# blachlylab/fade

Measured on NVIDIA B200. Metric: annotate_reads_per_sec, higher is better.
Workload: dtype int16

## Files before the change

### fade_b200/csrc/emu/emu.cu

```cuda
#include <cstdio>
#include <cstdlib>
#include <cstring>
#include <vector>
#include "../sw_core.cuh"

using namespace fade;

namespace {

template <int R>
struct ThreadState {
    uint32_t H[R], E[R], qs[R];
    uint32_t hu_prev, fout, M;
};

template <int R>
int align_pair(const uint8_t *qa, int qlen_a, const uint8_t *ta, int tlen_a,
               const uint8_t *qb, int qlen_b, const uint8_t *tb, int tlen_b,
               const SwConsts &k, int extra_blocks, int tagged, int32_t min_length,
               uint32_t clipl_a, uint32_t clipr_a, uint32_t clipl_b, uint32_t clipr_b,
               AlnOut *out_a, AlnOut *out_b)
{
    const int rows = FG * R;
    if (qlen_a > rows || qlen_b > rows) return -1;
    const int tmax = tlen_a > tlen_b ? tlen_a : tlen_b;
    const int nblk = num_blocks(tmax) + extra_blocks;
    const int TW = FBLK * nblk + FG + 1;
    std::vector<uint16_t> tw(TW);
    for (int idx = 0; idx < TW; ++idx) {
        const int j = idx - FG;
        const int ca = (j >= 0 && j < tlen_a) ? ta[j] : C_TPAD;
        const int cb = (j >= 0 && j < tlen_b) ? tb[j] : C_TPAD;
        tw[idx] = (uint16_t)t_sel(ca, cb);
    }
    std::vector<uint8_t> qc(rows);
    std::vector<ThreadState<R>> st(FG);
    for (int g = 0; g < FG; ++g)
        for (int r = 0; r < R; ++r) {
            const int i = g * R + r;
            const int ca = i < qlen_a ? qa[i] : C_QPAD;
            const int cb = i < qlen_b ? qb[i] : C_QPAD;
            st[g].qs[r] = q_sel(ca, cb);
            qc[i] = (uint8_t)(ca | (cb << 4));
        }
    auto init_state = [&](ThreadState<R> &s) {
        for (int r = 0; r < R; ++r) { s.H[r] = 0; s.E[r] = k.neg_o; }
        s.hu_prev = 0; s.fout = k.neg_o; s.M = 0;
    };
    for (int g = 0; g < FG; ++g) init_state(st[g]);

    const int CW = ck_words<R>();
    std::vector<uint32_t> ck((size_t)nblk * FG * CW);
    LaneCtl ctl[2];
    memset(ctl, 0, sizeof(ctl));
    uint32_t Mprev[FG];
    for (int g = 0; g < FG; ++g) Mprev[g] = 0;
    for (int c = 0; c < nblk; ++c) {
        for (int u = 0; u < FBLK; ++u) {
            const int t = c * FBLK + u;
            uint32_t hu[FG], fin[FG];
            for (int g = 0; g < FG; ++g) {
                hu[g] = g == 0 ? 0u : st[g - 1].H[R - 1];
                fin[g] = g == 0 ? k.neg_o : st[g - 1].fout;
            }
            for (int g = 0; g < FG; ++g) {
                const uint32_t ts = tw[t - g + FG];
                const uint32_t hd = st[g].hu_prev;
                fill_step<R>(st[g].H, st[g].E, st[g].qs, st[g].M, ts, hd, fin[g], st[g].fout, k);
                st[g].hu_prev = hu[g];
            }
        }
        for (int g = 0; g < FG; ++g) {
            uint32_t *p = &ck[((size_t)c * FG + g) * CW];
            for (int r = 0; r < R; ++r) { p[r] = st[g].H[r]; p[R + r] = st[g].E[r]; }
            p[2 * R] = st[g].hu_prev;
            p[2 * R + 1] = st[g].fout;
            if (st[g].M != Mprev[g]) {
                if (lane_lo(st[g].M) != lane_lo(Mprev[g])) ctl[0].blk[g] = c;
                if (lane_hi(st[g].M) != lane_hi(Mprev[g])) ctl[1].blk[g] = c;
                Mprev[g] = st[g].M;
            }
        }
    }
    for (int g = 0; g < FG; ++g) { ctl[0].best[g] = lane_lo(st[g].M); ctl[1].best[g] = lane_hi(st[g].M); }

    ctl_init(ctl[0], qlen_a, tlen_a);
    ctl_init(ctl[1], qlen_b, tlen_b);
    constexpr int RW = trace_words<R>();
    std::vector<uint32_t> tr((size_t)tile_words<R>());
    const bool tg = (tagged & 1) && k.tagged_ok;
    int guard = 0;
    bool first_iter = true;
    while (ctl[0].phase != 2 || ctl[1].phase != 2) {
        if (++guard > 4 * nblk + 16) return -2;
        int blk[2];
        for (int L = 0; L < 2; ++L) blk[L] = (ctl[L].phase != 2 && ctl[L].next_blk >= 0) ? ctl[L].next_blk : 0;
        bool scan[2][FG];
        for (int L = 0; L < 2; ++L)
            for (int g = 0; g < FG; ++g) scan[L][g] = (ctl_scanmask(ctl[L]) >> g) & 1u;
        for (int g = 0; g < FG; ++g) {
            ThreadState<R> s0, s1;
            init_state(s0); init_state(s1);
            auto load = [&](ThreadState<R> &s, int b) {
                if (b == 0) return;
                const uint32_t *p = &ck[((size_t)(b - 1) * FG + g) * CW];
                for (int r = 0; r < R; ++r) { s.H[r] = p[r]; s.E[r] = p[R + r]; }
                s.hu_prev = p[2 * R]; s.fout = p[2 * R + 1];
            };
            load(s0, blk[0]); load(s1, blk[1]);
            auto mix = [&](uint32_t a, uint32_t b) {
                const uint32_t w = (a & 0xffffu) | (b & 0xffff0000u);
                return tg ? to_tagged(w) : w;
            };
            for (int r = 0; r < R; ++r) { st[g].H[r] = mix(s0.H[r], s1.H[r]); st[g].E[r] = mix(s0.E[r], s1.E[r]); }
            st[g].hu_prev = mix(s0.hu_prev, s1.hu_prev);
            st[g].fout = mix(s0.fout, s1.fout);
        }
        const uint32_t f_top = tg ? k.neg_o16 : k.neg_o;
        const int mul = tg ? 16 : 1;
        bool found[2][FG];
        for (int L = 0; L < 2; ++L) for (int g = 0; g < FG; ++g) found[L][g] = false;
        for (int u = 0; u < FBLK; ++u) {
            const int t0 = blk[0] * FBLK + u, t1 = blk[1] * FBLK + u;
            uint32_t hu[FG], fin[FG];
            for (int g = 0; g < FG; ++g) {
                hu[g] = g == 0 ? 0u : st[g - 1].H[R - 1];
                fin[g] = g == 0 ? f_top : st[g - 1].fout;
            }
            for (int g = 0; g < FG; ++g) {
                const uint32_t ts = (tw[t0 - g + FG] & 0x00ffu) | (tw[t1 - g + FG] & 0xff00u);
                uint32_t cmax = 0;
                uint32_t trw[RW];
                if (tg) trace_step_tagged<R>(st[g].H, st[g].E, st[g].qs, ts, st[g].hu_prev, fin[g], st[g].fout, k, trw, cmax);
                else trace_step_plain<R>(st[g].H, st[g].E, st[g].qs, ts, st[g].hu_prev, fin[g], st[g].fout, k, trw, cmax);
                st[g].hu_prev = hu[g];
                for (int w = 0; w < RW; ++w) tr[(size_t)tile_index<R>(u, g, w)] = trw[w];
                for (int L = 0; L < 2; ++L) {
                    if (!scan[L][g] || found[L][g]) continue;
                    const int cm = L == 0 ? lane_lo(cmax) : lane_hi(cmax);
                    if (cm != ctl[L].S * mul) continue;
                    for (int r = 0; r < R; ++r) {
                        const int hv = L == 0 ? lane_lo(st[g].H[r]) : lane_hi(st[g].H[r]);
                        if (hv == ctl[L].S * mul) {
                            found[L][g] = true;
                            ctl[L].fj[g] = (L == 0 ? t0 : t1) - g;
                            ctl[L].fr[g] = r;
                            break;
                        }
                    }
                }
            }
        }
        for (int L = 0; L < 2; ++L)
            for (int g = 0; g < FG; ++g)
                if (scan[L][g] && !found[L][g]) return -3;
        const bool so0 = (tagged & 4) && ctl[0].phase == 0 && first_iter, so1 = (tagged & 4) && ctl[1].phase == 0 && first_iter;
        ctl_advance<R>(ctl[0], so0 ? nullptr : tr.data(), 0, StagedAcc{ tw.data(), qc.data(), 0 }, k);
        ctl_advance<R>(ctl[1], so1 ? nullptr : tr.data(), 1, StagedAcc{ tw.data(), qc.data(), 1 }, k);
        first_iter = false;
    }
    finalize_result(ctl[0], *out_a, 0, clipl_a, clipr_a, min_length);
    finalize_result(ctl[1], *out_b, 1, clipl_b, clipr_b, min_length);
    return 0;
}

}

extern "C" int fadeemu_align_pair(int R, const uint8_t *qa, int qlen_a, const uint8_t *ta, int tlen_a,
                                  const uint8_t *qb, int qlen_b, const uint8_t *tb, int tlen_b,
                                  int open, int extend, int match, int mismatch, int extra_blocks,
                                  int tagged, int min_length, const uint32_t *clips ,
                                  AlnOut *out_a, AlnOut *out_b)
{
    SwConsts k = make_consts(open, extend, match, mismatch);
    k.shortcut = (tagged & 2) ? 0 : 1;
#define CASE(RR)                                                                                   \
    case RR:                                                                                       \
        return align_pair<RR>(qa, qlen_a, ta, tlen_a, qb, qlen_b, tb, tlen_b, k, extra_blocks,    \
                              tagged, min_length, clips[0], clips[1], clips[2], clips[3], out_a, out_b);
    switch (R) {
        CASE(1) CASE(2) CASE(3) CASE(5) CASE(13) CASE(19) CASE(25) CASE(32) CASE(38)
    default: return -10;
    }
#undef CASE
}

extern "C" int fadeemu_comp_code_of_nt16(int nib) { return comp_code_of_nt16(nib); }
extern "C" uint32_t fadeemu_prmt(uint32_t a, uint32_t b, uint32_t s) { return prmt_sx(a, b, s); }
extern "C" int fadeemu_sizeof_alnout(void) { return (int)sizeof(AlnOut); }
```

### fade_b200/csrc/kernels.cu

```cuda
#include "kernels.cuh"
#include <algorithm>
#include <cstdio>
#include <cstdlib>

namespace fade {

namespace {

constexpr unsigned FULL = 0xffffffffu;

#define FADE_SMALL_KERNEL __launch_bounds__(128, 16)


__device__ __forceinline__ uint32_t stage_targets(const KernelArgs &a, const AlnDesc &da, const AlnDesc &db, int g,
                                                  int step0, int nsteps, uint16_t *tw)
{
    const int TW = nsteps + FG + 1;
    uint32_t w = 0;
    for (int idx = g; idx < TW; idx += FG) {
        const int j = step0 + idx - FG;
        int ca = C_TPAD, cb = C_TPAD;
        if (j >= 0 && j < da.tlen) ca = ref_code(a.ref.planes, da.gstart + j);
        if (j >= 0 && j < db.tlen) cb = ref_code(a.ref.planes, db.gstart + j);
        w |= (ca == C_WILD ? 1u : 0u) | (cb == C_WILD ? 2u : 0u);
        tw[idx] = (uint16_t)t_sel(ca, cb);
    }
    return w;
}

template <int R>
__device__ __forceinline__ void stage_pair(const KernelArgs &a, const AlnDesc &da, const AlnDesc &db,
                                           int g, int nblk, uint16_t *tw, uint32_t (&qs)[R],
                                           uint8_t *qc, uint32_t &wild)
{
    uint32_t w = stage_targets(a, da, db, g, 0, FBLK * min(nblk, FILL_CHUNK_BLOCKS), tw);
    const uint8_t *sa = a.seq + da.seq_off, *sb = a.seq + db.seq_off;
#pragma unroll
    for (int r = 0; r < R; ++r) {
        const int i = g * R + r;
        int ca = C_QPAD, cb = C_QPAD;
        if (i < da.qlen) ca = rc_query_code(sa, da.qlen, i);
        if (i < db.qlen) cb = rc_query_code(sb, db.qlen, i);
        w |= (ca == C_WILD ? 1u : 0u) | (cb == C_WILD ? 2u : 0u);
        qs[r] = q_sel(ca, cb);
        if (qc) qc[i] = (uint8_t)(ca | (cb << 4));
    }
    wild = w;
}

__device__ __forceinline__ AlnDesc load_desc(const KernelArgs &a, int idx)
{
    AlnDesc d;
    if (idx < a.n_aln) d = a.aln[idx];
    else { d.gstart = 0; d.seq_off = 0; d.tlen = 0; d.qlen = 0; d.clip_left = d.clip_right = 0; d.read = -1; d.pad = 0; }
    return d;
}

template <int R>
__global__ void __launch_bounds__(FILL_THREADS, (R <= 19 ? 5 : 1)) sw_fill_kernel(const KernelArgs a)
{
    extern __shared__ __align__(16) unsigned char smem_raw[];
    const int lane = threadIdx.x & 31, wib = threadIdx.x >> 5;
    const int g = lane & (FG - 1), q = lane >> 3;
    const int w = blockIdx.x * (FILL_THREADS / 32) + wib;
    if (w >= a.n_items) return;
    const WarpItem item = a.items[w];
    const int ia = item.first + 2 * q, ib = ia + 1;
    const AlnDesc da = load_desc(a, ia), db = load_desc(a, ib);
    uint16_t *tw = reinterpret_cast<uint16_t *>(smem_raw) + (size_t)(wib * 4 + q) * a.tw_stride;
    const int nblk = item.nblk;
    const SwConsts k = a.k;

    uint32_t H[R], E[R], qs[R];
    uint32_t wild;
    stage_pair<R>(a, da, db, g, nblk, tw, qs, nullptr, wild);
#pragma unroll
    for (int r = 0; r < R; ++r) { H[r] = 0u; E[r] = k.neg_o; }
    uint32_t hu_prev = 0u, fout = k.neg_o, M = 0u, Mprev = 0u;
    int blk_lo = 0, blk_hi = 0;
    __syncwarp();

    constexpr int CW = ck_words<R>();
    uint32_t *ckw = a.ck + item.ck_off + lane;
    const uint16_t *twp = tw + (FG - g);
    const int nsteps = item.nsteps;
    for (int c = 0; c < nblk; ++c) {
        if (c > 0 && (c % FILL_CHUNK_BLOCKS) == 0) {
            __syncwarp();
            wild |= stage_targets(a, da, db, g, c * FBLK, FBLK * min(nblk - c, FILL_CHUNK_BLOCKS), tw);
            twp = tw + (FG - g) - c * FBLK;
            __syncwarp();
        }
        const int ulim = min(FBLK, nsteps - c * FBLK);
#pragma unroll 2
        for (int u = 0; u < ulim; ++u) {
            const int t = c * FBLK + u;
            uint32_t hu = __shfl_up_sync(FULL, H[R - 1], 1, FG);
            uint32_t fin = __shfl_up_sync(FULL, fout, 1, FG);
            if (g == 0) { hu = 0u; fin = k.neg_o; }
            const uint32_t ts = twp[t];
            fill_step<R>(H, E, qs, M, ts, hu_prev, fin, fout, k);
            hu_prev = hu;
        }
        if (c + 1 < nblk) {
            uint32_t *p = ckw + (size_t)c * CW * 32;
#pragma unroll
            for (int r = 0; r < R; ++r) { p[r * 32] = H[r]; p[(R + r) * 32] = E[r]; }
            p[(2 * R) * 32] = hu_prev;
            p[(2 * R + 1) * 32] = fout;
        }
        if (M != Mprev) {
            if ((M ^ Mprev) & 0xffffu) blk_lo = c;
            if ((M ^ Mprev) >> 16) blk_hi = c;
            Mprev = M;
        }
    }
    a.fillres[(size_t)w * 32 + lane] = make_uint2(M, (uint32_t)blk_lo | ((uint32_t)blk_hi << 16));
    if ((wild & 1u) && ia < a.n_aln) a.aln_flags[ia] = 1u;
    if ((wild & 2u) && ib < a.n_aln) a.aln_flags[ib] = 1u;
}

__device__ __forceinline__ unsigned long long pack_req(int aln, int blk, uint32_t scanmask)
{
    return (unsigned long long)(uint32_t)aln | ((unsigned long long)(uint32_t)(blk & 0xffff) << 32) |
           ((unsigned long long)(scanmask & 0xffu) << 48);
}

struct GlobalAcc {
    const uint8_t *seq;
    int qlen;
    RefPlanes planes;
    int64_t gstart;
    __device__ __forceinline__ int qcode(int i) const { return rc_query_code(seq, qlen, i); }
    __device__ __forceinline__ int tcode(int j) const { return ref_code(planes, gstart + j); }
};

template <int R>
__global__ void FADE_SMALL_KERNEL trace_init_kernel(const KernelArgs a)
{
    for (int aln = blockIdx.x * blockDim.x + threadIdx.x; aln < a.n_aln; aln += gridDim.x * blockDim.x) {
        a.out[aln].read = -1;
        a.out[aln].flags = 0x80000000u;
        if (a.aln_flags[aln] & 1u) continue;
        const AlnDesc d = a.aln[aln];
        LaneCtl &c = a.state[aln];
        const int w = aln >> 3, q = (aln & 7) >> 1, half = aln & 1;
        const uint2 *fr = a.fillres + (size_t)w * 32 + q * FG;
        for (int g = 0; g < FG; ++g) {
            const uint2 v = fr[g];
            c.best[g] = half ? lane_hi(v.x) : lane_lo(v.x);
            c.blk[g] = half ? (int)(v.y >> 16) : (int)(v.y & 0xffffu);
        }
        ctl_init(c, d.qlen, d.tlen);
        if (c.phase != 2 && a.tags_only && !score_may_accept(c.S, d.clip_left, d.clip_right, a.min_length)) {
            AlnOut o;
            o.score = c.S; o.end_query = o.end_ref = o.beg_query = o.beg_ref = 0; o.n_ops = 0;
            o.flags = R_ALIGNED | R_SCORE_ONLY; o.read = d.read;
            for (int k = 0; k < OPS_CAP; ++k) o.ops[k] = 0;
            a.out[aln] = o;
        } else if (c.phase == 2) {
            AlnOut o;
            finalize_result(c, o, d.read, d.clip_left, d.clip_right, a.min_length);
            a.out[aln] = o;
        } else {
            const unsigned slot = atomicAdd(&a.qcount[0], 1u);
            a.queue[0][slot] = pack_req(aln, c.next_blk, ctl_scanmask(c));
        }
    }
}

template <int R, int MODE>
__device__ __forceinline__ void replay_round(const KernelArgs &a, int round, unsigned warp0, unsigned nwarps,
                                             uint16_t (*tws_all)[40])
{
    constexpr bool TAGGED = MODE == 0;
    constexpr bool SCAN_ONLY = MODE == 2;
    constexpr int RW = trace_words<R>();
    constexpr int CW = ck_words<R>();
    constexpr int MUL = TAGGED ? 16 : 1;
    const int lane = threadIdx.x & 31, wib = threadIdx.x >> 5;
    const int g = lane & (FG - 1), q = lane >> 3;
    const int rin = round & 1;
    const unsigned cnt = a.qcount[rin];
    const unsigned long long *queue = a.queue[rin];
    const unsigned npairs = (cnt + 1u) >> 1;
    const unsigned nquads = (npairs + 3u) >> 2;
    const SwConsts k = a.k;
    const uint32_t e_init = TAGGED ? k.neg_o16 : k.neg_o;
    uint16_t *tws = tws_all[wib * 4 + q];
    for (unsigned quad = warp0; quad < nquads; quad += nwarps) {
        const unsigned pair = quad * 4u + (unsigned)q;
        int aln[2], blk[2], half[2], S[2];
        uint32_t smask[2];
        AlnDesc d[2];
        const uint32_t *ckp[2];
#pragma unroll
        for (int L = 0; L < 2; ++L) {
            const unsigned ri = pair * 2u + (unsigned)L;
            if (ri < cnt) {
                const unsigned long long rq = queue[ri];
                aln[L] = (int)(uint32_t)(rq & 0xffffffffu);
                blk[L] = (int)((rq >> 32) & 0xffffu);
                smask[L] = (uint32_t)((rq >> 48) & 0xffu);
                d[L] = a.aln[aln[L]];
                const WarpItem it = a.items[aln[L] >> 3];
                ckp[L] = a.ck + it.ck_off + (((aln[L] & 7) >> 1) * FG + g);
                half[L] = aln[L] & 1;
                S[L] = a.state[aln[L]].S * MUL;
            } else {
                aln[L] = -1; blk[L] = 0; smask[L] = 0; half[L] = 0; S[L] = -1; ckp[L] = a.ck;
                d[L].gstart = 0; d[L].seq_off = 0; d[L].tlen = 0; d[L].qlen = 0;
            }
        }
        uint32_t H[R], E[R], qs[R], hu_prev, fout;
        {
            const uint32_t *p0 = ckp[0] + (size_t)(blk[0] > 0 ? blk[0] - 1 : 0) * CW * 32;
            const uint32_t *p1 = ckp[1] + (size_t)(blk[1] > 0 ? blk[1] - 1 : 0) * CW * 32;
            const bool z0 = blk[0] == 0, z1 = blk[1] == 0;
            const int sh0 = half[0] * 16, sh1 = half[1] * 16;
            auto mix = [&](uint32_t w0, uint32_t w1) {
                const uint32_t w = ((w0 >> sh0) & 0xffffu) | ((w1 >> sh1) << 16);
                return TAGGED ? to_tagged(w) : w;
            };
#pragma unroll
            for (int r = 0; r < R; ++r) {
                H[r] = mix(z0 ? 0u : p0[r * 32], z1 ? 0u : p1[r * 32]);
                E[r] = mix(z0 ? k.neg_o : p0[(R + r) * 32], z1 ? k.neg_o : p1[(R + r) * 32]);
            }
            hu_prev = mix(z0 ? 0u : p0[(2 * R) * 32], z1 ? 0u : p1[(2 * R) * 32]);
            fout = mix(z0 ? k.neg_o : p0[(2 * R + 1) * 32], z1 ? k.neg_o : p1[(2 * R + 1) * 32]);
        }
        {
            const uint8_t *s0 = a.seq + d[0].seq_off, *s1 = a.seq + d[1].seq_off;
#pragma unroll
            for (int r = 0; r < R; ++r) {
                const int i = g * R + r;
                const int ca = i < d[0].qlen ? rc_query_code(s0, d[0].qlen, i) : C_QPAD;
                const int cb = i < d[1].qlen ? rc_query_code(s1, d[1].qlen, i) : C_QPAD;
                qs[r] = q_sel(ca, cb);
            }
            __syncwarp();
            for (int x = g; x < FBLK + FG - 1; x += FG) {
                const int j0 = blk[0] * FBLK - (FG - 1) + x, j1 = blk[1] * FBLK - (FG - 1) + x;
                const int ca = (j0 >= 0 && j0 < d[0].tlen) ? ref_code(a.ref.planes, d[0].gstart + j0) : C_TPAD;
                const int cb = (j1 >= 0 && j1 < d[1].tlen) ? ref_code(a.ref.planes, d[1].gstart + j1) : C_TPAD;
                tws[x] = (uint16_t)t_sel(ca, cb);
            }
            __syncwarp();
        }
        uint32_t *tile = a.tiles + (size_t)pair * tile_words<R>();
        const bool store = aln[0] >= 0;
        bool need0 = (smask[0] >> g) & 1u, need1 = (smask[1] >> g) & 1u;
        const uint16_t *twp = tws + (FG - 1 - g);
        for (int u = 0; u < FBLK; ++u) {
            uint32_t hu = __shfl_up_sync(FULL, H[R - 1], 1, FG);
            uint32_t fin = __shfl_up_sync(FULL, fout, 1, FG);
            if (g == 0) { hu = 0u; fin = e_init; }
            const uint32_t ts = twp[u];
            uint32_t cmax = 0u;
            if (SCAN_ONLY) {
                fill_step<R>(H, E, qs, cmax, ts, hu_prev, fin, fout, k);
            } else {
                uint32_t trw[RW];
                if (TAGGED) trace_step_tagged<R>(H, E, qs, ts, hu_prev, fin, fout, k, trw, cmax);
                else trace_step_plain<R>(H, E, qs, ts, hu_prev, fin, fout, k, trw, cmax);
                if (store) {
#pragma unroll
                    for (int w = 0; w < RW; ++w) tile[tile_index<R>(u, g, w)] = trw[w];
                }
            }
            hu_prev = hu;
            if (need0 && lane_lo(cmax) == S[0]) {
                need0 = false;
                int fr = 0;
#pragma unroll
                for (int r = R - 1; r >= 0; --r) if (lane_lo(H[r]) == S[0]) fr = r;
                a.state[aln[0]].fj[g] = blk[0] * FBLK + u - g;
                a.state[aln[0]].fr[g] = fr;
            }
            if (need1 && lane_hi(cmax) == S[1]) {
                need1 = false;
                int fr = 0;
#pragma unroll
                for (int r = R - 1; r >= 0; --r) if (lane_hi(H[r]) == S[1]) fr = r;
                a.state[aln[1]].fj[g] = blk[1] * FBLK + u - g;
                a.state[aln[1]].fr[g] = fr;
            }
            if (SCAN_ONLY && !__any_sync(FULL, need0 || need1)) break;
        }
    }
}

template <int R, int MODE>
__global__ void __launch_bounds__(128) trace_replay_kernel(const KernelArgs a)
{
    __shared__ uint16_t tws_all[16][40];
    if (blockIdx.x == 0 && threadIdx.x == 0) a.qcount[(a.round & 1) ^ 1] = 0u;
    replay_round<R, MODE>(a, a.round, blockIdx.x * (blockDim.x >> 5) + (threadIdx.x >> 5),
                            gridDim.x * (blockDim.x >> 5), tws_all);
}

struct AdvanceSmem {
    LaneCtl ctl;
    AlnOut out;
};
static_assert(sizeof(LaneCtl) % 4 == 0 && sizeof(AlnOut) % 4 == 0, "word-copyable");

template <int R>
__device__ __forceinline__ void advance_round(const KernelArgs &a, int round, unsigned warp0, unsigned nwarps,
                                              AdvanceSmem *smem_all)
{
    constexpr int RW = trace_words<R>();
    constexpr int CTLW = (int)(sizeof(LaneCtl) / 4), OUTW = (int)(sizeof(AlnOut) / 4);
    AdvanceSmem &sm = smem_all[threadIdx.x >> 5];
    const int rin = round & 1;
    const unsigned cnt = a.qcount[rin];
    const unsigned long long *queue = a.queue[rin];
    const int l = threadIdx.x & 31;
    const SwConsts &k = a.k;
    const bool tile_valid = !(round == 0 && k.shortcut);
    for (unsigned idx = warp0; idx < cnt; idx += nwarps) {
        const int aln = (int)(uint32_t)(queue[idx] & 0xffffffffu);
        const AlnDesc d = a.aln[aln];
        LaneCtl &c = sm.ctl;
        {
            const uint32_t *src = reinterpret_cast<const uint32_t *>(&a.state[aln]);
            uint32_t *dst = reinterpret_cast<uint32_t *>(&c);
            for (int w = l; w < CTLW; w += 32) dst[w] = src[w];
        }
        __syncwarp();
        const uint32_t *tile = a.tiles + (size_t)(idx >> 1) * tile_words<R>();
        const int sh = 16 * (int)(idx & 1u);
        GlobalAcc acc;
        acc.seq = a.seq + d.seq_off; acc.qlen = d.qlen; acc.planes = a.ref.planes; acc.gstart = d.gstart;
        int go = 1;
        if (l == 0) {
            c.cur_blk = c.next_blk;
            if (c.phase == 0 && !ctl_select_end<R>(c)) go = 0;
        }
        go = __shfl_sync(FULL, go, 0);
        __syncwarp();
        bool done = false;
        int need = -1;
        if (go) {
            int i = 0, j = 0, mode = 0, hval = 0, gval = 0, nrev = 0, cur_blk_ = 0;
            uint32_t cur = 0;
            if (l == 0) {
                i = c.i; j = c.j; mode = c.mode; hval = c.hval; gval = c.gval; nrev = c.nrev; cur = c.cur;
                cur_blk_ = c.cur_blk;
            }
            i = __shfl_sync(FULL, i, 0); j = __shfl_sync(FULL, j, 0); mode = __shfl_sync(FULL, mode, 0);
            hval = __shfl_sync(FULL, hval, 0); gval = __shfl_sync(FULL, gval, 0); nrev = __shfl_sync(FULL, nrev, 0);
            cur = __shfl_sync(FULL, cur, 0);
            const int cur_blk = __shfl_sync(FULL, cur_blk_, 0);
            auto push_n = [&](uint32_t op, int n) {
                if (cur != 0 && (cur & 0xf) == op) { cur += 16u * (uint32_t)n; return; }
                if (cur != 0) { if (l == 0) c.ring[nrev % OPS_CAP] = cur; ++nrev; }
                cur = ((uint32_t)n << 4) | op;
            };
            int forced = 0;
            for (;;) {
                if (i < 0 || j < 0) { done = true; break; }
                if (mode == 0 && hval <= 0) { done = true; break; }
                if (mode == 0) {
                    const int ii = i - l, jj = j - l;
                    const bool valid = ii >= 0 && jj >= 0;
                    const int g = valid ? ii / R : 0, r = valid ? ii - g * R : 0;
                    const int t = jj + g;
                    const bool inblk = valid && tile_valid && (t / FBLK) == cur_blk;
                    uint32_t nib = 0;
                    int sc = 0;
                    bool eq = false;
                    if (valid && (inblk || forced > 0)) {
                        eq = acc.qcode(ii) == acc.tcode(jj);
                        sc = eq ? k.match : k.mismatch;
                    }
                    if (inblk && forced == 0)
                        nib = (tile[tile_index<R>(t % FBLK, g, r >> 2)] >> (sh + 4 * (r & 3))) & 0xfu;
                    const bool diag = forced > 0 ? (valid && l < forced) : (inblk && (nib >> 2) == 2u);
                    if (!diag) sc = 0;
                    int pre = sc;
// ... 367 lines not shown
        if (tmax_g) atomicMax(&a.stats[5], (unsigned long long)tmax_g);
        if (bad) atomicOr(&a.stats[6], bad);
        if (fetched) atomicAdd(&a.stats[10], (unsigned long long)fetched);
    }
}

__global__ void FADE_SMALL_KERNEL bin_scatter_kernel(const BinArgs a)
{
    for (int64_t r = (int64_t)blockIdx.x * blockDim.x + threadIdx.x; r < a.n; r += (int64_t)gridDim.x * blockDim.x) {
        const int key = a.key[r];
        if (key < 0) continue;
        const int slot = a.keybase[key] + atomicAdd(&a.cursor[key], 1);
        AlnDesc d;
        d.gstart = a.coff[a.tid[r]] + a.start[r];
        d.seq_off = a.seq_off[r];
        if (a.seq_cursor) {
            const int64_t so = d.seq_off;
            const int ph = (int)(so & 15);
            const unsigned long long bytes = (unsigned long long)((ph + (a.l_qseq[r] + 1) / 2 + 15) & ~15);
            d.seq_off = (int64_t)atomicAdd(a.seq_cursor, bytes) + ph;
            a.src_off[slot] = so;
        }
        d.tlen = a.tlen[r];
        d.qlen = a.l_qseq[r];
        d.clip_left = (uint32_t)a.clip_left[r];
        d.clip_right = (uint32_t)a.clip_right[r];
        d.read = a.read ? a.read[r] : (int32_t)r;
        d.pad = 0;
        a.aln[slot] = d;
        a.aln_start[slot] = a.start[r];
    }
}

__global__ void FADE_SMALL_KERNEL seq_pull_kernel(const uint8_t *__restrict__ host_seq4, const AlnDesc *__restrict__ aln,
                                                       const int64_t *__restrict__ src_off, int n_aln, uint8_t *__restrict__ dst)
{
    const int lane = threadIdx.x & 7;
    for (int k = (blockIdx.x * blockDim.x + threadIdx.x) >> 3; k < n_aln; k += (gridDim.x * blockDim.x) >> 3) {
        const int64_t so = src_off[k];
        const int ph = (int)(so & 15);
        const int chunks = (ph + (aln[k].qlen + 1) / 2 + 15) >> 4;
        const uint4 *s = reinterpret_cast<const uint4 *>(host_seq4 + (so - ph));
        uint4 *d = reinterpret_cast<uint4 *>(dst + (aln[k].seq_off - ph));
        for (int i = lane; i < chunks; i += 8) d[i] = s[i];
    }
}

__global__ void FADE_SMALL_KERNEL result_index_kernel(const AlnOut *out, int n_aln, int64_t n_reads, uint8_t *flags, int32_t *ridx,
                                                      unsigned long long *n_ok)
{
    int ok = 0;
    for (int k = blockIdx.x * blockDim.x + threadIdx.x; k < n_aln; k += gridDim.x * blockDim.x) {
        const int r = out[k].read;
        const uint32_t f = out[k].flags;
        if (r >= 0 && (int64_t)r < n_reads && (f & 1u) && !(f & 0x80000000u)) { flags[r] = (uint8_t)(f & 0xffu); ridx[r] = k; ++ok; }
    }
    ok = __reduce_add_sync(FULL, ok);
    if ((threadIdx.x & 31) == 0 && ok) atomicAdd(n_ok, (unsigned long long)ok);
}

__global__ void __launch_bounds__(256) alu_peak_kernel(uint32_t *out, int iters)
{
    uint32_t x0 = threadIdx.x, x1 = x0 + 1, x2 = x0 + 2, x3 = x0 + 3, x4 = x0 + 4, x5 = x0 + 5, x6 = x0 + 6, x7 = x0 + 7;
    const uint32_t c = 0x00010003u + blockIdx.x, d = 0xfffefffdu;
    for (int i = 0; i < iters; ++i) {
#pragma unroll
        for (int u = 0; u < 8; ++u) {
            x0 = __viaddmax_s16x2(x0, c, d); x1 = __viaddmax_s16x2(x1, c, d);
            x2 = __viaddmax_s16x2(x2, c, d); x3 = __viaddmax_s16x2(x3, c, d);
            x4 = __viaddmax_s16x2(x4, c, d); x5 = __viaddmax_s16x2(x5, c, d);
            x6 = __viaddmax_s16x2(x6, c, d); x7 = __viaddmax_s16x2(x7, c, d);
        }
    }
    const uint32_t r = x0 ^ x1 ^ x2 ^ x3 ^ x4 ^ x5 ^ x6 ^ x7;
    if (r == 0x12345678u) out[0] = r;
}

}

int tw_stride_for(int nblk_max) { return (FBLK * std::min(nblk_max, FILL_CHUNK_BLOCKS) + FG + 1 + 7) & ~7; }

size_t fill_smem_bytes(int tw_stride) { return (size_t)(FILL_THREADS / FG) * tw_stride * 2; }

template <int R>
static cudaError_t launch_fill_t(const KernelArgs &a, cudaStream_t s)
{
    const size_t smem = fill_smem_bytes(a.tw_stride);
    cudaError_t e = cudaFuncSetAttribute(sw_fill_kernel<R>, cudaFuncAttributeMaxDynamicSharedMemorySize, (int)smem);
    if (e != cudaSuccess) return e;
    const int wpb = FILL_THREADS / 32;
    const int grid = (a.n_items + wpb - 1) / wpb;
    sw_fill_kernel<R><<<grid, FILL_THREADS, smem, s>>>(a);
    return cudaGetLastError();
}

template <int R, bool TAGGED>
static cudaError_t launch_trace_tt(KernelArgs a, cudaStream_t s, int sm_count, int *launches)
{
    const int n = a.n_aln;
    int grid = std::min((n + 127) / 128, sm_count * 8);
    trace_init_kernel<R><<<grid, 128, 0, s>>>(a);
    int nl = 1;
    constexpr int FULL_ROUNDS = 10;
    const int quads = (n + 7) / 8;
    int r = 0;
    for (; r < a.max_rounds && r < FULL_ROUNDS; ++r) {
        a.round = r;
        const int g1 = std::min((quads + 3) / 4, r < 3 ? sm_count * 4 : sm_count);
        const int g2 = std::min((n + 3) / 4, r < 3 ? sm_count * 16 : sm_count * 2);
        if (getenv("FADEGPU_DEBUG_ROUNDS")) {
            unsigned int qc[2] = { 0, 0 };
            cudaStreamSynchronize(s);
            cudaMemcpy(qc, a.qcount, sizeof(qc), cudaMemcpyDeviceToHost);
            fprintf(stderr, "[fadegpu] round %d: %u requests (n_aln %d)\n", r, qc[r & 1], n);
        }
        if (r == 0 && a.k.shortcut) trace_replay_kernel<R, 2><<<std::max(g1, 1), 128, 0, s>>>(a);
        else trace_replay_kernel<R, TAGGED ? 0 : 1><<<std::max(g1, 1), 128, 0, s>>>(a);
        trace_advance_kernel<R><<<std::max(g2, 1), 128, 0, s>>>(a);
        nl += 2;
    }
    if (r < a.max_rounds) {
        a.round = r;
        trace_tail_kernel<R, TAGGED><<<1, 128, 0, s>>>(a);
        nl += 1;
    }
    if (launches) *launches += nl;
    return cudaGetLastError();
}

template <int R>
static cudaError_t launch_trace_t(const KernelArgs &a, cudaStream_t s, int sm_count, int *launches)
{
    return a.k.tagged_ok ? launch_trace_tt<R, true>(a, s, sm_count, launches)
                         : launch_trace_tt<R, false>(a, s, sm_count, launches);
}

cudaError_t launch_fill(int R, const KernelArgs &a, cudaStream_t s)
{
    if (a.n_items <= 0) return cudaSuccess;
    switch (R) {
    case 13: return launch_fill_t<13>(a, s);
    case 19: return launch_fill_t<19>(a, s);
    case 25: return launch_fill_t<25>(a, s);
    case 32: return launch_fill_t<32>(a, s);
    case 38: return launch_fill_t<38>(a, s);
    default: return cudaErrorInvalidValue;
    }
}

cudaError_t launch_trace(int R, const KernelArgs &a, cudaStream_t s, int sm_count, int *launches)
{
    if (a.n_items <= 0) return cudaSuccess;
    switch (R) {
    case 13: return launch_trace_t<13>(a, s, sm_count, launches);
    case 19: return launch_trace_t<19>(a, s, sm_count, launches);
    case 25: return launch_trace_t<25>(a, s, sm_count, launches);
    case 32: return launch_trace_t<32>(a, s, sm_count, launches);
    case 38: return launch_trace_t<38>(a, s, sm_count, launches);
    default: return cudaErrorInvalidValue;
    }
}

size_t trace_tile_bytes(int R)
{
    switch (R) {
    case 13: return (size_t)tile_words<13>() * 4;
    case 19: return (size_t)tile_words<19>() * 4;
    case 25: return (size_t)tile_words<25>() * 4;
    case 32: return (size_t)tile_words<32>() * 4;
    default: return (size_t)tile_words<38>() * 4;
    }
}

cudaError_t launch_bin_classify(const BinArgs &a, int sm_count, cudaStream_t s)
{
    if (a.n <= 0) return cudaSuccess;
    const int grid = (int)std::min<int64_t>((a.n + 127) / 128, (int64_t)sm_count * 16);
    bin_classify_kernel<<<grid, 128, 0, s>>>(a);
    return cudaGetLastError();
}

cudaError_t launch_bin_scatter(const BinArgs &a, int sm_count, cudaStream_t s)
{
    if (a.n <= 0) return cudaSuccess;
    const int grid = (int)std::min<int64_t>((a.n + 127) / 128, (int64_t)sm_count * 16);
    bin_scatter_kernel<<<grid, 128, 0, s>>>(a);
    return cudaGetLastError();
}

cudaError_t launch_seq_pull(const uint8_t *host_seq4, const AlnDesc *aln, const int64_t *src_off, int n_aln, uint8_t *dst, int sm_count,
                            cudaStream_t s)
{
    if (n_aln <= 0) return cudaSuccess;
    const int grid = std::min((n_aln * 8 + 127) / 128, sm_count * 16);
    seq_pull_kernel<<<grid, 128, 0, s>>>(host_seq4, aln, src_off, n_aln, dst);
    return cudaGetLastError();
}

cudaError_t launch_result_index(const AlnOut *out, int n_aln, int64_t n_reads, uint8_t *flags, int32_t *ridx, unsigned long long *n_ok,
// ... 25 lines not shown
```

### fade_b200/csrc/sw_core.cuh

```cuda
#pragma once
#include <stdint.h>

#if defined(__CUDACC__)
#define FD __host__ __device__ __forceinline__
#else
#define FD inline
#endif

namespace fade {

constexpr int FG = 8;
constexpr int FBLK = 32;
constexpr int OPS_CAP = 10;

enum : int { C_A = 0, C_C = 1, C_T = 2, C_G = 3, C_N = 4, C_WILD = 5, C_TPAD = 6, C_QPAD = 7 };

enum : uint32_t { OP_I = 1, OP_D = 2, OP_S = 4, OP_EQ = 7, OP_X = 8 };

struct SwConsts {
    uint32_t lut0, lut1;
    uint32_t neg_o, neg_e;
    int32_t open, extend, match, mismatch;
    uint32_t tlut0, tlut1;
    uint32_t neg_o16;
    uint32_t neg_e16_e;
    uint32_t neg_e16_f;
    int32_t tagged_ok;
    int32_t shortcut;
};

FD SwConsts make_consts(int open, int extend, int match, int mismatch)
{
    SwConsts k;
    const uint32_t m = (uint32_t)(match & 0xff), x = (uint32_t)(mismatch & 0xff);
    k.lut0 = m | (x << 8) | (x << 16) | (x << 24);
    k.lut1 = x | (x << 8) | (x << 16) | (x << 24);
    const uint32_t no = (uint32_t)((-open) & 0xffff), ne = (uint32_t)((-extend) & 0xffff);
    k.neg_o = no | (no << 16);
    k.neg_e = ne | (ne << 16);
    k.open = open; k.extend = extend; k.match = match; k.mismatch = mismatch;
    const int tm = 16 * match + 8, tx = 16 * mismatch + 8;
    k.tagged_ok = (tm <= 127 && tx >= -128 && open <= 1000) ? 1 : 0;
    const uint32_t bm = (uint32_t)(tm & 0xff), bx = (uint32_t)(tx & 0xff);
    k.tlut0 = bm | (bx << 8) | (bx << 16) | (bx << 24);
    k.tlut1 = bx | (bx << 8) | (bx << 16) | (bx << 24);
    const uint32_t o16 = (uint32_t)((-16 * open) & 0xffff);
    const uint32_t ee = (uint32_t)((-16 * extend + 1) & 0xffff), ef = (uint32_t)((-16 * extend + 2) & 0xffff);
    k.neg_o16 = o16 | (o16 << 16);
    k.neg_e16_e = ee | (ee << 16);
    k.neg_e16_f = ef | (ef << 16);
    k.shortcut = 1;
    return k;
}

FD int lane_lo(uint32_t w) { return (int)(int16_t)(w & 0xffffu); }
FD int lane_hi(uint32_t w) { return (int)(int16_t)(w >> 16); }
FD uint32_t pack2(int lo, int hi) { return ((uint32_t)lo & 0xffffu) | ((uint32_t)hi << 16); }

FD uint32_t prmt_sx(uint32_t a, uint32_t b, uint32_t sel)
{
#if defined(__CUDA_ARCH__)
    uint32_t d;
    asm("prmt.b32 %0, %1, %2, %3;" : "=r"(d) : "r"(a), "r"(b), "r"(sel));
    return d;
#else
    const uint64_t v = ((uint64_t)b << 32) | a;
    uint32_t d = 0;
    for (int i = 0; i < 4; ++i) {
        const uint32_t c = (sel >> (4 * i)) & 0xf;
        uint32_t byte = (uint32_t)(v >> (8 * (c & 7))) & 0xff;
        if (c & 8) byte = (byte & 0x80) ? 0xff : 0x00;
        d |= byte << (8 * i);
    }
    return d;
#endif
}

FD uint32_t q_sel(int ca, int cb) { return (uint32_t)(ca * 0x11) | ((uint32_t)(cb * 0x11) << 8); }
FD uint32_t t_sel(int ca, int cb) { return (uint32_t)(ca * 0x11 | 0x80) | ((uint32_t)(cb * 0x11 | 0x80) << 8); }
FD uint32_t score_word(uint32_t qs, uint32_t ts, const SwConsts &k) { return prmt_sx(k.lut0, k.lut1, qs ^ ts); }

struct RefPlanes {
    const uint32_t *two;
    const uint32_t *nmask;
    const uint32_t *xmask;
};

FD int ref_code(const RefPlanes &rp, int64_t p)
{
    const uint32_t w = rp.two[p >> 4];
    int c = (int)((w >> (2 * (int)(p & 15))) & 3u);
    if ((rp.nmask[p >> 5] >> (int)(p & 31)) & 1u) c = C_N;
    if ((rp.xmask[p >> 5] >> (int)(p & 31)) & 1u) c = C_WILD;
    return c;
}

FD int nt16_at(const uint8_t *seq4, int i) { return (seq4[i >> 1] >> ((~i & 1) << 2)) & 0xf; }

FD int comp_code_of_nt16(int nib)
{
    const uint64_t lut = 0x4555555055515325ull;
    return (int)((lut >> (4 * nib)) & 0xf);
}

FD int rc_query_code(const uint8_t *seq4, int qlen, int i)
{
    return comp_code_of_nt16(nt16_at(seq4, qlen - 1 - i));
}

FD uint32_t FADE_VADD(uint32_t a, uint32_t b)
{
#if defined(__CUDA_ARCH__)
    return __vadd2(a, b);
#else
    return pack2(lane_lo(a) + lane_lo(b), lane_hi(a) + lane_hi(b));
#endif
}
FD uint32_t FADE_VMAX(uint32_t a, uint32_t b)
{
#if defined(__CUDA_ARCH__)
    return __vmaxs2(a, b);
#else
    const int l = lane_lo(a) > lane_lo(b) ? lane_lo(a) : lane_lo(b);
    const int h = lane_hi(a) > lane_hi(b) ? lane_hi(a) : lane_hi(b);
    return pack2(l, h);
#endif
}
FD uint32_t FADE_VMAX3(uint32_t a, uint32_t b, uint32_t c)
{
#if defined(__CUDA_ARCH__)
    return __vimax3_s16x2(a, b, c);
#else
    return FADE_VMAX(FADE_VMAX(a, b), c);
#endif
}
FD uint32_t FADE_VIADDMAX(uint32_t a, uint32_t b, uint32_t c)
{
#if defined(__CUDA_ARCH__)
    return __viaddmax_s16x2(a, b, c);
#else
    return FADE_VMAX(FADE_VADD(a, b), c);
#endif
}
FD uint32_t FADE_VIADDMAX_RELU(uint32_t a, uint32_t b, uint32_t c)
{
#if defined(__CUDA_ARCH__)
    return __viaddmax_s16x2_relu(a, b, c);
#else
    return FADE_VMAX(FADE_VIADDMAX(a, b, c), 0u);
#endif
}

template <int R>
FD void fill_step(uint32_t (&H)[R], uint32_t (&E)[R], const uint32_t (&qs)[R], uint32_t &M,
                  uint32_t ts, uint32_t hdiag, uint32_t f_in, uint32_t &f_out, const SwConsts &k)
{
    uint32_t f = f_in;
#pragma unroll
    for (int r = 0; r < R; ++r) {
        const uint32_t s = score_word(qs[r], ts, k);
        const uint32_t t1 = FADE_VIADDMAX_RELU(hdiag, s, E[r]);
        const uint32_t h = FADE_VMAX(t1, f);
        hdiag = H[r];
        H[r] = h;
        const uint32_t ho = FADE_VADD(h, k.neg_o);
        E[r] = FADE_VIADDMAX(E[r], k.neg_e, ho);
        f = FADE_VIADDMAX(f, k.neg_e, ho);
        M = FADE_VMAX(M, h);
    }
    f_out = f;
}

template <int R> FD constexpr int trace_words() { return (R + 3) / 4; }

FD uint32_t trace_nibble_plain(int d0, int ev, int fv, int h, int o, int e)
{
    uint32_t nib = (h == d0) ? 8u : ((h == fv) ? 4u : 0u);
    if (!(h - o > ev - e)) nib |= 1u;
    if (!(h - o > fv - e)) nib |= 2u;
    return nib;
}

template <int R>
FD void trace_step_plain(uint32_t (&H)[R], uint32_t (&E)[R], const uint32_t (&qs)[R],
                         uint32_t ts, uint32_t hdiag, uint32_t f_in, uint32_t &f_out, const SwConsts &k,
                         uint32_t *trw, uint32_t &cmax)
{
    uint32_t f = f_in, acc = 0;
#pragma unroll
    for (int r = 0; r < R; ++r) {
        const uint32_t s = score_word(qs[r], ts, k);
        const uint32_t d0 = FADE_VIADDMAX_RELU(hdiag, s, 0u);
        const uint32_t ev = E[r];
        const uint32_t h = FADE_VMAX(FADE_VMAX(d0, ev), f);
        const uint32_t nl = trace_nibble_plain(lane_lo(d0), lane_lo(ev), lane_lo(f), lane_lo(h), k.open, k.extend);
        const uint32_t nh = trace_nibble_plain(lane_hi(d0), lane_hi(ev), lane_hi(f), lane_hi(h), k.open, k.extend);
        acc |= (nl | (nh << 16)) << (4 * (r & 3));
        if ((r & 3) == 3 || r == R - 1) { trw[r >> 2] = acc; acc = 0; }
        hdiag = H[r];
        H[r] = h;
        cmax = FADE_VMAX(cmax, h);
        const uint32_t ho = FADE_VADD(h, k.neg_o);
        E[r] = FADE_VIADDMAX(ev, k.neg_e, ho);
        f = FADE_VIADDMAX(f, k.neg_e, ho);
    }
    f_out = f;
}

template <int R>
FD void trace_step_tagged(uint32_t (&H)[R], uint32_t (&E)[R], const uint32_t (&qs)[R],
                          uint32_t ts, uint32_t hdiag, uint32_t f_in, uint32_t &f_out, const SwConsts &k,
                          uint32_t *trw, uint32_t &cmax)
{
    uint32_t f = f_in, acc = 0;
#pragma unroll
    for (int r = 0; r < R; ++r) {
        const uint32_t s16 = prmt_sx(k.tlut0, k.tlut1, qs[r] ^ ts);
        const uint32_t t1 = FADE_VIADDMAX_RELU(hdiag, s16, E[r]);
        const uint32_t hv = FADE_VIADDMAX(f, 0x00040004u, t1);
        const uint32_t hc = hv & 0xfff0fff0u;
        hdiag = H[r];
        H[r] = hc;
        cmax = FADE_VMAX(cmax, hc);
        const uint32_t ho = FADE_VADD(hc, k.neg_o16);
        const uint32_t en = FADE_VIADDMAX(E[r] & 0xfff0fff0u, k.neg_e16_e, ho);
        const uint32_t fn = FADE_VIADDMAX(f & 0xfff0fff0u, k.neg_e16_f, ho);
        E[r] = en;
        f = fn;
        const uint32_t nib = (hv & 0x000c000cu) | ((en | fn) & 0x00030003u);
        acc += nib << (4 * (r & 3));
        if ((r & 3) == 3 || r == R - 1) { trw[r >> 2] = acc; acc = 0; }
    }
    f_out = f;
}

FD uint32_t to_tagged(uint32_t w) { return (w << 4) & 0xfff0fff0u; }


enum : int { T_ZERO = 0, T_DIAG = 1, T_F = 2, T_E = 3, T_EOPEN = 4, T_FOPEN = 8 };

template <int R>
FD void locate(int i, int j, int &blk, int &u)
{
    const int g = i / R;
    const int t = j + g;
// ... 234 lines not shown
```

Baseline: 229.4 million.

## Compute diagonal score add via f16x2 FMA on integer bit patterns in fill

Adds an alternate fill step that forms hdiag+score with an fma.rn.f16x2 on the raw int16 bit patterns, using denormal arithmetic with a specially encoded score LUT, then takes a three-way max with ReLU. This moves the add off the integer SIMD pipe onto the FP16 FMA pipe to balance issue load. A host-side exactness check over the reachable value range gates the path per scoring scheme. It adds F16 template variants of the fill and scan-only replay kernels, plus emulator hooks for testing.

```diff
diff --git a/fade_b200/csrc/emu/emu.cu b/fade_b200/csrc/emu/emu.cu
--- a/fade_b200/csrc/emu/emu.cu
+++ b/fade_b200/csrc/emu/emu.cu
@@ -10,7 +10,7 @@
 
 template <int R>
 struct ThreadState {
-    uint32_t H[R], E[R], qs[R];
+    uint32_t H[R], E[R], qs[R], qf[R];
     uint32_t hu_prev, fout, M;
 };
 
@@ -41,6 +41,7 @@
             const int ca = i < qlen_a ? qa[i] : C_QPAD;
             const int cb = i < qlen_b ? qb[i] : C_QPAD;
             st[g].qs[r] = q_sel(ca, cb);
+            st[g].qf[r] = q_self(ca, cb);
             qc[i] = (uint8_t)(ca | (cb << 4));
         }
     auto init_state = [&](ThreadState<R> &s) {
@@ -49,6 +50,7 @@
     };
     for (int g = 0; g < FG; ++g) init_state(st[g]);
 
+    const bool f16 = k.f16_ok && !(tagged & 8);
     const int CW = ck_words<R>();
     std::vector<uint32_t> ck((size_t)nblk * FG * CW);
     LaneCtl ctl[2];
@@ -66,7 +68,8 @@
             for (int g = 0; g < FG; ++g) {
                 const uint32_t ts = tw[t - g + FG];
                 const uint32_t hd = st[g].hu_prev;
-                fill_step<R>(st[g].H, st[g].E, st[g].qs, st[g].M, ts, hd, fin[g], st[g].fout, k);
+                if (f16) fill_step_f16<R>(st[g].H, st[g].E, st[g].qf, st[g].M, ts, hd, fin[g], st[g].fout, k);
+                else fill_step<R>(st[g].H, st[g].E, st[g].qs, st[g].M, ts, hd, fin[g], st[g].fout, k);
                 st[g].hu_prev = hu[g];
             }
         }
@@ -188,3 +191,8 @@
 extern "C" int fadeemu_comp_code_of_nt16(int nib) { return comp_code_of_nt16(nib); }
 extern "C" uint32_t fadeemu_prmt(uint32_t a, uint32_t b, uint32_t s) { return prmt_sx(a, b, s); }
 extern "C" int fadeemu_sizeof_alnout(void) { return (int)sizeof(AlnOut); }
+extern "C" int fadeemu_f16_ok(int open, int extend, int match, int mismatch) { return make_consts(open, extend, match, mismatch).f16_ok; }
+extern "C" void fadeemu_fma_f16x2(const uint32_t *a, const uint32_t *b, const uint32_t *c, uint32_t *out, int64_t n)
+{
+    for (int64_t i = 0; i < n; ++i) out[i] = fma_f16x2(a[i], b[i], c[i]);
+}
diff --git a/fade_b200/csrc/kernels.cu b/fade_b200/csrc/kernels.cu
--- a/fade_b200/csrc/kernels.cu
+++ b/fade_b200/csrc/kernels.cu
@@ -28,7 +28,7 @@
     return w;
 }
 
-template <int R>
+template <int R, bool F16>
 __device__ __forceinline__ void stage_pair(const KernelArgs &a, const AlnDesc &da, const AlnDesc &db,
                                            int g, int nblk, uint16_t *tw, uint32_t (&qs)[R],
                                            uint8_t *qc, uint32_t &wild)
@@ -42,7 +42,7 @@
         if (i < da.qlen) ca = rc_query_code(sa, da.qlen, i);
         if (i < db.qlen) cb = rc_query_code(sb, db.qlen, i);
         w |= (ca == C_WILD ? 1u : 0u) | (cb == C_WILD ? 2u : 0u);
-        qs[r] = q_sel(ca, cb);
+        qs[r] = F16 ? q_self(ca, cb) : q_sel(ca, cb);
         if (qc) qc[i] = (uint8_t)(ca | (cb << 4));
     }
     wild = w;
@@ -56,7 +56,15 @@
     return d;
 }
 
-template <int R>
+template <int R, bool F16>
+__device__ __forceinline__ void score_step(uint32_t (&H)[R], uint32_t (&E)[R], const uint32_t (&qs)[R], uint32_t &M,
+                                           uint32_t ts, uint32_t hdiag, uint32_t f_in, uint32_t &f_out, const SwConsts &k)
+{
+    if (F16) fill_step_f16<R>(H, E, qs, M, ts, hdiag, f_in, f_out, k);
+    else fill_step<R>(H, E, qs, M, ts, hdiag, f_in, f_out, k);
+}
+
+template <int R, bool F16>
 __global__ void __launch_bounds__(FILL_THREADS, (R <= 19 ? 5 : 1)) sw_fill_kernel(const KernelArgs a)
 {
     extern __shared__ __align__(16) unsigned char smem_raw[];
@@ -73,7 +81,7 @@
 
     uint32_t H[R], E[R], qs[R];
     uint32_t wild;
-    stage_pair<R>(a, da, db, g, nblk, tw, qs, nullptr, wild);
+    stage_pair<R, F16>(a, da, db, g, nblk, tw, qs, nullptr, wild);
 #pragma unroll
     for (int r = 0; r < R; ++r) { H[r] = 0u; E[r] = k.neg_o; }
     uint32_t hu_prev = 0u, fout = k.neg_o, M = 0u, Mprev = 0u;
@@ -99,7 +107,7 @@
             uint32_t fin = __shfl_up_sync(FULL, fout, 1, FG);
             if (g == 0) { hu = 0u; fin = k.neg_o; }
             const uint32_t ts = twp[t];
-            fill_step<R>(H, E, qs, M, ts, hu_prev, fin, fout, k);
+            score_step<R, F16>(H, E, qs, M, ts, hu_prev, fin, fout, k);
             hu_prev = hu;
         }
         if (c + 1 < nblk) {
@@ -169,7 +177,7 @@
     }
 }
 
-template <int R, int MODE>
+template <int R, int MODE, bool F16 = false>
 __device__ __forceinline__ void replay_round(const KernelArgs &a, int round, unsigned warp0, unsigned nwarps,
                                              uint16_t (*tws_all)[40])
 {
@@ -237,7 +245,7 @@
                 const int i = g * R + r;
                 const int ca = i < d[0].qlen ? rc_query_code(s0, d[0].qlen, i) : C_QPAD;
                 const int cb = i < d[1].qlen ? rc_query_code(s1, d[1].qlen, i) : C_QPAD;
-                qs[r] = q_sel(ca, cb);
+                qs[r] = F16 ? q_self(ca, cb) : q_sel(ca, cb);
             }
             __syncwarp();
             for (int x = g; x < FBLK + FG - 1; x += FG) {
@@ -259,7 +267,7 @@
             const uint32_t ts = twp[u];
             uint32_t cmax = 0u;
             if (SCAN_ONLY) {
-                fill_step<R>(H, E, qs, cmax, ts, hu_prev, fin, fout, k);
+                score_step<R, F16>(H, E, qs, cmax, ts, hu_prev, fin, fout, k);
             } else {
                 uint32_t trw[RW];
                 if (TAGGED) trace_step_tagged<R>(H, E, qs, ts, hu_prev, fin, fout, k, trw, cmax);
@@ -291,12 +299,12 @@
     }
 }
 
-template <int R, int MODE>
+template <int R, int MODE, bool F16 = false>
 __global__ void __launch_bounds__(128) trace_replay_kernel(const KernelArgs a)
 {
     __shared__ uint16_t tws_all[16][40];
     if (blockIdx.x == 0 && threadIdx.x == 0) a.qcount[(a.round & 1) ^ 1] = 0u;
-    replay_round<R, MODE>(a, a.round, blockIdx.x * (blockDim.x >> 5) + (threadIdx.x >> 5),
+    replay_round<R, MODE, F16>(a, a.round, blockIdx.x * (blockDim.x >> 5) + (threadIdx.x >> 5),
                             gridDim.x * (blockDim.x >> 5), tws_all);
 }
 
@@ -830,16 +838,22 @@
 
 size_t fill_smem_bytes(int tw_stride) { return (size_t)(FILL_THREADS / FG) * tw_stride * 2; }
 
-template <int R>
-static cudaError_t launch_fill_t(const KernelArgs &a, cudaStream_t s)
+template <int R, bool F16>
+static cudaError_t launch_fill_tf(const KernelArgs &a, cudaStream_t s)
 {
     const size_t smem = fill_smem_bytes(a.tw_stride);
-    cudaError_t e = cudaFuncSetAttribute(sw_fill_kernel<R>, cudaFuncAttributeMaxDynamicSharedMemorySize, (int)smem);
+    cudaError_t e = cudaFuncSetAttribute(sw_fill_kernel<R, F16>, cudaFuncAttributeMaxDynamicSharedMemorySize, (int)smem);
     if (e != cudaSuccess) return e;
     const int wpb = FILL_THREADS / 32;
     const int grid = (a.n_items + wpb - 1) / wpb;
-    sw_fill_kernel<R><<<grid, FILL_THREADS, smem, s>>>(a);
+    sw_fill_kernel<R, F16><<<grid, FILL_THREADS, smem, s>>>(a);
     return cudaGetLastError();
+}
+
+template <int R>
+static cudaError_t launch_fill_t(const KernelArgs &a, cudaStream_t s)
+{
+    return a.k.f16_ok ? launch_fill_tf<R, true>(a, s) : launch_fill_tf<R, false>(a, s);
 }
 
 template <int R, bool TAGGED>
@@ -862,7 +876,10 @@
             cudaMemcpy(qc, a.qcount, sizeof(qc), cudaMemcpyDeviceToHost);
             fprintf(stderr, "[fadegpu] round %d: %u requests (n_aln %d)\n", r, qc[r & 1], n);
         }
-        if (r == 0 && a.k.shortcut) trace_replay_kernel<R, 2><<<std::max(g1, 1), 128, 0, s>>>(a);
+        if (r == 0 && a.k.shortcut) {
+            if (a.k.f16_ok) trace_replay_kernel<R, 2, true><<<std::max(g1, 1), 128, 0, s>>>(a);
+            else trace_replay_kernel<R, 2, false><<<std::max(g1, 1), 128, 0, s>>>(a);
+        }
         else trace_replay_kernel<R, TAGGED ? 0 : 1><<<std::max(g1, 1), 128, 0, s>>>(a);
         trace_advance_kernel<R><<<std::max(g2, 1), 128, 0, s>>>(a);
         nl += 2;
diff --git a/fade_b200/csrc/sw_core.cuh b/fade_b200/csrc/sw_core.cuh
--- a/fade_b200/csrc/sw_core.cuh
+++ b/fade_b200/csrc/sw_core.cuh
@@ -27,7 +27,116 @@
     uint32_t neg_e16_f;
     int32_t tagged_ok;
     int32_t shortcut;
+    uint32_t flut0, flut1;
+    int32_t f16_ok;
 };
+
+FD int lane_lo(uint32_t w) { return (int)(int16_t)(w & 0xffffu); }
+FD int lane_hi(uint32_t w) { return (int)(int16_t)(w >> 16); }
+FD uint32_t pack2(int lo, int hi) { return ((uint32_t)lo & 0xffffu) | ((uint32_t)hi << 16); }
+
+FD uint32_t prmt_sx(uint32_t a, uint32_t b, uint32_t sel)
+{
+#if defined(__CUDA_ARCH__)
+    uint32_t d;
+    asm("prmt.b32 %0, %1, %2, %3;" : "=r"(d) : "r"(a), "r"(b), "r"(sel));
+    return d;
+#else
+    const uint64_t v = ((uint64_t)b << 32) | a;
+    uint32_t d = 0;
+    for (int i = 0; i < 4; ++i) {
+        const uint32_t c = (sel >> (4 * i)) & 0xf;
+        uint32_t byte = (uint32_t)(v >> (8 * (c & 7))) & 0xff;
+        if (c & 8) byte = (byte & 0x80) ? 0xff : 0x00;
+        d |= byte << (8 * i);
+    }
+    return d;
+#endif
+}
+
+FD uint32_t q_sel(int ca, int cb) { return (uint32_t)(ca * 0x11) | ((uint32_t)(cb * 0x11) << 8); }
+FD uint32_t t_sel(int ca, int cb) { return (uint32_t)(ca * 0x11 | 0x80) | ((uint32_t)(cb * 0x11 | 0x80) << 8); }
+FD uint32_t score_word(uint32_t qs, uint32_t ts, const SwConsts &k) { return prmt_sx(k.lut0, k.lut1, qs ^ ts); }
+
+FD uint32_t f16_fma_lane(uint32_t a, uint32_t b, uint32_t c)
+{
+    struct Dec { int neg, m, e; };
+    auto dec = [](uint32_t x) {
+        const int ex = (int)((x >> 10) & 31), fr = (int)(x & 1023);
+        return Dec{ (int)((x >> 15) & 1), ex ? (fr | 1024) : fr, ex ? ex - 1 : 0 };
+    };
+    const Dec da = dec(a), db = dec(b), dc = dec(c);
+    const __int128 p = (__int128)((int64_t)da.m * db.m) << (da.e + db.e);
+    const __int128 q = (__int128)dc.m << (dc.e + 24);
+    const __int128 v = ((da.neg ^ db.neg) ? -p : p) + (dc.neg ? -q : q);
+    if (v == 0) return (p == 0 && q == 0 && (da.neg ^ db.neg) && dc.neg) ? 0x8000u : 0u;
+    const uint32_t sign = v < 0 ? 0x8000u : 0u;
+    const __int128 av = v < 0 ? -v : v;
+    int e = 0;
+    while (e < 30 && (av >> (24 + e)) >= 2048) ++e;
+    const int sh = 24 + e;
+    __int128 m = av >> sh;
+    const __int128 rem = av - (m << sh), half = (__int128)1 << (sh - 1);
+    if (rem > half || (rem == half && (m & 1))) ++m;
+    if (m == 2048) { m = 1024; ++e; }
+    if (e > 29) return sign | 0x7c00u;
+    if (m < 1024) return sign | (uint32_t)m;
+    return sign | ((uint32_t)(e + 1) << 10) | (uint32_t)(m - 1024);
+}
+
+FD uint32_t fma_f16x2(uint32_t a, uint32_t b, uint32_t c)
+{
+#if defined(__CUDA_ARCH__)
+    uint32_t d;
+    asm("fma.rn.f16x2 %0, %1, %2, %3;" : "=r"(d) : "r"(a), "r"(b), "r"(c));
+    return d;
+#else
+    return f16_fma_lane(a & 0xffffu, b & 0xffffu, c & 0xffffu) | (f16_fma_lane(a >> 16, b >> 16, c >> 16) << 16);
+#endif
+}
+
+constexpr uint32_t F16_UNIT = 0x00010001u;
+
+FD uint32_t q_self(int ca, int cb) { return (uint32_t)(ca * 0x11 | 0x88) | ((uint32_t)(cb * 0x11 | 0x88) << 8); }
+FD uint32_t score_word_f16(uint32_t qs, uint32_t ts, const SwConsts &k) { return prmt_sx(k.flut0, k.flut1, qs ^ ts); }
+
+FD int64_t f16_byte_word_x2(uint32_t b)
+{
+    const uint32_t w = b < 0x80 ? (b << 8) : ((b << 8) | 0xffu);
+    const int ex = (int)((w >> 10) & 31), fr = (int)(w & 1023);
+    const int64_t mag = ex ? (int64_t)(fr | 1024) << ex : (int64_t)fr * 2;
+    return (w & 0x8000u) ? -mag : mag;
+}
+
+FD uint32_t f16_score_byte(int v)
+{
+    uint32_t best = 0;
+    int64_t bd = -1;
+    for (uint32_t b = 0; b < 256; ++b) {
+        if ((b & 0x7c) == 0x7c) continue;
+        const int64_t d = f16_byte_word_x2(b) - ((int64_t)v << 25);
+        const int64_t ad = d < 0 ? -d : d;
+        if (bd < 0 || ad < bd) { bd = ad; best = b; }
+    }
+    return best;
+}
+
+FD bool f16_step_exact(const SwConsts &k)
+{
+    const int top = (k.match > k.mismatch ? k.match : k.mismatch) * FG * 38;
+    if (top > 2047) return false;
+    const int sc[2] = { k.match, k.mismatch };
+    const uint32_t sel[2] = { q_self(0, 0) ^ t_sel(0, 0), q_self(0, 0) ^ t_sel(1, 1) };
+    for (int n = 0; n <= top; ++n) {
+        for (int i = 0; i < 2; ++i) {
+            const int want = n + sc[i];
+            const uint32_t s = prmt_sx(k.flut0, k.flut1, sel[i]);
+            const uint32_t d = fma_f16x2(s, F16_UNIT, (uint32_t)n * 0x10001u);
+            if (want >= 0 ? d != (uint32_t)want * 0x10001u : (lane_lo(d) > 0 || lane_hi(d) > 0)) return false;
+        }
+    }
+    return true;
+}
 
 FD SwConsts make_consts(int open, int extend, int match, int mismatch)
 {
@@ -50,35 +159,12 @@
     k.neg_e16_e = ee | (ee << 16);
     k.neg_e16_f = ef | (ef << 16);
     k.shortcut = 1;
+    const uint32_t fm = f16_score_byte(match), fx = f16_score_byte(mismatch);
+    k.flut0 = fm | (fx << 8) | (fx << 16) | (fx << 24);
+    k.flut1 = fx | (fx << 8) | (fx << 16) | (fx << 24);
+    k.f16_ok = f16_step_exact(k) ? 1 : 0;
     return k;
 }
-
-FD int lane_lo(uint32_t w) { return (int)(int16_t)(w & 0xffffu); }
-FD int lane_hi(uint32_t w) { return (int)(int16_t)(w >> 16); }
-FD uint32_t pack2(int lo, int hi) { return ((uint32_t)lo & 0xffffu) | ((uint32_t)hi << 16); }
-
-FD uint32_t prmt_sx(uint32_t a, uint32_t b, uint32_t sel)
-{
-#if defined(__CUDA_ARCH__)
-    uint32_t d;
-    asm("prmt.b32 %0, %1, %2, %3;" : "=r"(d) : "r"(a), "r"(b), "r"(sel));
-    return d;
-#else
-    const uint64_t v = ((uint64_t)b << 32) | a;
-    uint32_t d = 0;
-    for (int i = 0; i < 4; ++i) {
-        const uint32_t c = (sel >> (4 * i)) & 0xf;
-        uint32_t byte = (uint32_t)(v >> (8 * (c & 7))) & 0xff;
-        if (c & 8) byte = (byte & 0x80) ? 0xff : 0x00;
-        d |= byte << (8 * i);
-    }
-    return d;
-#endif
-}
-
-FD uint32_t q_sel(int ca, int cb) { return (uint32_t)(ca * 0x11) | ((uint32_t)(cb * 0x11) << 8); }
-FD uint32_t t_sel(int ca, int cb) { return (uint32_t)(ca * 0x11 | 0x80) | ((uint32_t)(cb * 0x11 | 0x80) << 8); }
-FD uint32_t score_word(uint32_t qs, uint32_t ts, const SwConsts &k) { return prmt_sx(k.lut0, k.lut1, qs ^ ts); }
 
 struct RefPlanes {
     const uint32_t *two;
@@ -161,6 +247,34 @@
         const uint32_t s = score_word(qs[r], ts, k);
         const uint32_t t1 = FADE_VIADDMAX_RELU(hdiag, s, E[r]);
         const uint32_t h = FADE_VMAX(t1, f);
+        hdiag = H[r];
+        H[r] = h;
+        const uint32_t ho = FADE_VADD(h, k.neg_o);
+        E[r] = FADE_VIADDMAX(E[r], k.neg_e, ho);
+        f = FADE_VIADDMAX(f, k.neg_e, ho);
+        M = FADE_VMAX(M, h);
+    }
+    f_out = f;
+}
+
+FD uint32_t FADE_VMAX3_RELU(uint32_t a, uint32_t b, uint32_t c)
+{
+#if defined(__CUDA_ARCH__)
+    return __vimax3_s16x2_relu(a, b, c);
+#else
+    return FADE_VMAX(FADE_VMAX3(a, b, c), 0u);
+#endif
+}
+
+template <int R>
+FD void fill_step_f16(uint32_t (&H)[R], uint32_t (&E)[R], const uint32_t (&qs)[R], uint32_t &M,
+                      uint32_t ts, uint32_t hdiag, uint32_t f_in, uint32_t &f_out, const SwConsts &k)
+{
+    uint32_t f = f_in;
+#pragma unroll
+    for (int r = 0; r < R; ++r) {
+        const uint32_t d = fma_f16x2(score_word_f16(qs[r], ts, k), F16_UNIT, hdiag);
+        const uint32_t h = FADE_VMAX3_RELU(d, E[r], f);
         hdiag = H[r];
         H[r] = h;
         const uint32_t ho = FADE_VADD(h, k.neg_o);
```

Measured after the change: 249.8 million, median of 6. 1.09x the previous value.
